# lukechencqu/quadrupedal_foothold_planner

Hardware: AMD Instinct MI355X
Metric: footholds/sec (4 legs x N cycles x B poses) on 1k^2 @2cm map; `value` = device-resident (poses and every product stay in HBM), `value_8d` / `ms_per_step_8d` = SURVEY 8(d)'s wall time of fpe_plan with host buffers, result D2H included (pinned destinations; pageable ones in value_survey_8d) (higher is better)
Workload: dtype f64; 1 GPU; headline: 1000x1000 @2cm rough terrain (seed 1), B=4096 poses/GPU (seed 6), trot, 8 cycles, searchRadius 0.1, all products written; `value` is device-resident (inputs and results stay in HBM; the PCIe-inclusive rate is value_incl_d2h); poses_per_gpu=4096, n_cycles=8, generator=synth-1, kernels=bit-window where supported, exchange=none

## Files before the change

### quadrupedal_foothold_planner_amd/csrc/fpe_bits_lane8.hpp

```cpp
#pragma once

namespace {


struct Unit {
    float eA[9];
    float eB[9];
    float eC;
    uint32_t pad0;
    uint32_t visA, visB;
    int nomRow, nomCol;
    uint32_t nomFlags;
    int cenRow, cenCol;
    uint32_t cenCode;
    double cx;
    double cenX;
    double defX;
    uint32_t pad[2];
};
static_assert(sizeof(Unit) == 144 && sizeof(Unit) % 16 == 0 && offsetof(Unit, visA) == 80 && offsetof(Unit, cx) == 112, "Unit layout");

template <bool kWant>
__device__ __forceinline__ void unit_put_disc(const DevMap& m, const PlanConsts& pc, double cx, double cy, const BBox& bb,
                                              const Grp<8>& g, const DiscLoads& d, float* e, uint32_t& vis, float* scratch) {
// ... 320 lines not shown
        c.xlo = nx2 - r;
        c.yhi = ny + 0.5 * r;
        c.ylo = ny - 0.5 * r;
    }
    c.vx = sh.polyX[leg];
    c.vy = sh.polyY[leg];
    c.footDa = sh.footDa;
    c.footDb = sh.footDb;
    c.footOff = sh.footOff;
    c.R2 = lk.R2;
    c.nRings = lk.nRings;
    c.nCand = lk.nCand;
    c.ti0 = c.tj0 = 0;
    c.ici = c.icj = 0;

    NominalOut no;
    CentroidOut co;
    float zDefault = static_cast<float>(static_cast<double>(0.0f) + pc.h);
    float* scratch = reinterpret_cast<float*>(lb.a);
    const bool wantDefault = out.default_next != nullptr;
    const bool usable = (ye.flags & 2) != 0 && fabs(c.cx) <= 1e6;
    if (!ls.radiusOk || !usable) {
        nominal_invalid(no, c.cx, c.cy, ls.radiusOk ? 2 : 3);
        co.x = co.y = 0.0; co.z = 0.0f; co.row = co.col = -1; co.code = 6;
        if (wantDefault && centre_usable(nx0, ny)) {
            const BBox dbox = circle_bbox_fast(m.g, nx0, ny, pc.rf);
            bool unused;
            zDefault = disc_pass_direct<G, false>(m, pc, nx0, ny, dbox, g, unused, scratch);
        }
        if constexpr (kMid) {
            if (g.sub == 0) {
                unit->visA = 0x80000000u;
                unit->eA[0] = 0.0f;
                unit->visB = 0x80000000u;
                unit->eB[0] = zDefault;
                unit->eC = 0.0f;
            }
        } else {
            ugFlags = kUgPreA | kUgPreB;
            ugVisA = __float_as_uint(0.0f);
            ugVisB = __float_as_uint(zDefault);
        }
    } else {
        const int q = g.sub;
        const double cq = (q == 5 || q == 6) ? nx0 : c.cx;
        const bool rawq = q == 4 || q == 7;
        const double hq = (q == 2 || q == 3) ? 0.5 * lk.lx : (rawq ? 0.0 : pc.rf);
        const bool minus = q == 1 || q == 3 || q == 6;
        const double xq = rawq ? cq : (minus ? cq - hq : cq + hq);
        int idxq;
        bool withinq = true;
        {
            const double n = (xq - m.g.orgX) - m.g.posX;
            const double qf = n * m.g.rinv;
            const double k = trunc(qf);
            const double fr = fabs(qf - k);
            bool safe = fr > pc.cornerEps && fr < 1.0 - pc.cornerEps;
            if (!rawq) safe = safe && qf < -pc.cornerEps && qf > pc.cornerEps - static_cast<double>(m.g.rows);
            idxq = -static_cast<int>(k);
            if (__ballot(!safe) != 0ull) {
                const Box bq{cq, 0.0, hq, 0.0};
                const CornerVal cv = corner_quantity(m.g, minus ? 2 : 0, bq, rawq);
                idxq = cv.idx;
                withinq = cv.within;
            }
        }
        constexpr int kKeep = (~(G - 1)) & 0x1F;
        BBox bb, rbox, dbox;
        bb.i0 = __builtin_amdgcn_ds_swizzle(idxq, kKeep | (0 << 5));
        bb.ni = __builtin_amdgcn_ds_swizzle(idxq, kKeep | (1 << 5)) - bb.i0 + 1;
        rbox.i0 = __builtin_amdgcn_ds_swizzle(idxq, kKeep | (2 << 5));
        rbox.ni = __builtin_amdgcn_ds_swizzle(idxq, kKeep | (3 << 5)) - rbox.i0 + 1;
        c.ici = __builtin_amdgcn_ds_swizzle(idxq, kKeep | (4 << 5));
        dbox.i0 = __builtin_amdgcn_ds_swizzle(idxq, kKeep | (5 << 5));
        dbox.ni = __builtin_amdgcn_ds_swizzle(idxq, kKeep | (6 << 5)) - dbox.i0 + 1;
        bb.j0 = dbox.j0 = ye.j0d;
        bb.nj = dbox.nj = ye.njd;
        rbox.j0 = ye.j0r;
        rbox.nj = ye.njr;
        c.icj = ye.jc;
        const unsigned wbits = static_cast<unsigned>(g.ballot(withinq));
        Submap sm;
        sm.i0 = rbox.i0;
        sm.j0 = rbox.j0;
        sm.ni = rbox.ni;
        sm.nj = rbox.nj;
        {
            const bool okX = (wbits & 0xCu) == 0xCu && sm.i0 >= 0 && sm.i0 < m.g.rows && sm.i0 + sm.ni <= m.g.rows;
            const double cornerX = cell_pos(m.g.baseX, m.g.res, sm.i0) - (-(0.5 * m.g.res));
            const double subLenX = static_cast<double>(sm.ni) * m.g.res;
            const double subOrgX = 0.5 * subLenX;
            const double subPosX = cornerX - subOrgX;
            sm.ok = okX && (ye.flags & 1) != 0 && within_axis(c.cx, subOrgX, subPosX, subLenX);
            sm.baseX = sm.ok ? subPosX + (subOrgX - 0.5 * m.g.res) : 0.0;
            sm.baseY = sm.ok ? ye.sbaseY : 0.0;
        }
        const int iw0 = c.ici - pc.winH, jw0 = c.icj - pc.winH;
        uint4 grp[NRL][KW + 1];
        win_issue<G, NRL, KW>(bm, m.g, g, iw0, jw0, grp);
        DiscLoads dc, dd;
        const bool dfltUsable = wantDefault && fabs(nx0) <= 1e6;
        uint32_t rowA = 0u, rowB = 0u;
        bool rowsA = false, rowsB = false;
        if constexpr (kMid) {
            disc_issue<G, false, kMid, kMid>(m, pc, c.cx, c.cy, bb, g, dc, ye.dy2);
            if (dfltUsable) disc_issue<G, false, kMid, kMid>(m, pc, nx0, ny, dbox, g, dd, ye.dy2);
        } else {
            dc.pipelined = dd.pipelined = false;
            dc.mid = dd.mid = false;
            const bool fitA = bb.ni <= 8 && bb.nj <= 8 && bb.ni * bb.nj <= 32;
            const bool fitB = !dfltUsable || (dbox.ni <= 8 && dbox.nj <= 8 && dbox.ni * dbox.nj <= 32);
            rowsA = __ballot(!fitA) == 0ull;
            rowsB = __ballot(!fitB) == 0ull;
            if (rowsA || rowsB) disc_rows8(m.g, pc.rf2, c.cx, nx0, c.cy, bb, dbox, g, rowA, rowB);
        }
        WinRows<NRL, KW> w;
        win_finish<NRL, KW>(jw0, grp, w);
#pragma unroll
        for (int k = 0; k < NRL; ++k) lb.a[g.sub + G * k] = w.Df[k][0];
        const CentroidScan sc = rows_from_bits<G, NRL, KW>(sm, w, g, iw0, jw0);
        bits_sync<G>();
        bool defaultOk;
        if constexpr (kMid) {
            defaultOk = default_ok_bits<G, KW, kMid>(m, pc, c.cx, c.cy, bb, dc, lb.a, lb.rows, iw0, jw0, g);
        } else {
            defaultOk = rowsA ? default_ok_rows8(rowA, bb, lb.a, lb.rows, iw0, jw0, g)
                              : default_ok_bits<G, KW, kMid>(m, pc, c.cx, c.cy, bb, dc, lb.a, lb.rows, iw0, jw0, g);
        }
        bits_sync<G>();
        float zCentre = 0.0f;
        if constexpr (kMid) {
            uint32_t visA = 0u, visB = 0u;
            unit_put_disc<true>(m, pc, c.cx, c.cy, bb, g, dc, unit->eA, visA, scratch);
            if (dfltUsable) unit_put_disc<true>(m, pc, nx0, ny, dbox, g, dd, unit->eB, visB, scratch);
            if (g.sub == 0) {
                unit->visA = visA;
                unit->visB = visB;
            }
        } else {
            bool pre;
            if (rowsA) {
                ugVisA = box_mask_from_rows8(rowA, bb.nj, g);
            } else {
                unitg_put_disc(m, pc, c.cx, c.cy, bb, g, dc, ugVisA, pre, scratch);
                if (pre) ugFlags |= kUgPreA;
            }
            ugAI0 = bb.i0; ugAJ0 = bb.j0; ugANj = max(bb.nj, 1);
            if (dfltUsable) {
                if (rowsB) {
                    ugVisB = box_mask_from_rows8(rowB, dbox.nj, g);
                } else {
                    unitg_put_disc(m, pc, nx0, ny, dbox, g, dd, ugVisB, pre, scratch);
                    if (pre) ugFlags |= kUgPreB;
                }
                ugBI0 = dbox.i0; ugBJ0 = dbox.j0; ugBNj = max(dbox.nj, 1);
            } else {
                ugFlags |= kUgPreB;
                ugVisB = __float_as_uint(zDefault);
            }
        }
        constexpr bool kOneCell = kMid;
        CentroidPendingBits cp;
        centroid_begin_bits<kOneCell>(m, c, sm, sc, zCentre, cp, ye.yA, ye.yB);
        if (defaultOk) {
            no.valid = 1;
            no.source = 0;
            no.row = c.ici;
            no.col = c.icj;
            no.x = c.cx;
            no.y = c.cy;
            no.z = zCentre;
        } else {
            nominal_invalid(no, c.cx, c.cy, 2);
            int wi = 0, wj = 0;
            bits_sync<G>();
            if (spiral_bits<G, NRL, KW, kMid>(m, pc, lut, head, c, w, lb, g, iw0, jw0, wi, wj, &ye)) {
                no.valid = 1;
                no.source = 1;
                no.row = wi;
                no.col = wj;
                no.x = cell_pos(m.g.baseX, m.g.res, wi);
                no.y = cell_pos(m.g.baseY, m.g.res, wj);
                no.z = zCentre;
            }
            bits_sync<G>();
        }
        if constexpr (kMid) {
            if (g.sub == 0) unit->eC = cp.e0;
            cp.o.z = 0.0f;
            if (g.sub == 0) unit->cenCode = static_cast<uint32_t>(cp.o.code) | (cp.needDisc != 0 ? 0x100u : 0u);
        } else {
            cp.o.z = 0.0f;
            if (cp.needDisc != 0) ugFlags |= kUgCTable;
            else if (cp.o.code == 0) ugFlags |= kUgCIsA;
        }
        co = cp.o;
    }
    lc->valid = no.valid;
    lc->v[0][0] = nx0;   lc->v[0][1] = ny;    lc->v[0][2] = static_cast<double>(zDefault);
    lc->v[1][0] = co.x;  lc->v[1][1] = co.y;  lc->v[1][2] = static_cast<double>(co.z);
    lc->v[2][0] = no.x;  lc->v[2][1] = no.y;  lc->v[2][2] = static_cast<double>(no.z);
    if constexpr (!kMid) {
        if (g.sub == 0) {
            UnitG u;
            u.cx = c.cx; u.cenX = co.x; u.defX = nx0;
            u.aI0 = ugAI0; u.aJ0 = ugAJ0; u.visA = ugVisA;
            u.bI0 = ugBI0; u.bJ0 = ugBJ0; u.visB = ugVisB;
            u.nomRow = no.row; u.nomCol = no.col; u.cenRow = co.row; u.cenCol = co.col;
            u.flags = static_cast<uint32_t>(co.code) | (no.valid ? kUgValid : 0u) | (static_cast<uint32_t>(no.source) << kUgSrcShift) | ugFlags |
                      (static_cast<uint32_t>(ugANj) << 16) | (static_cast<uint32_t>(ugBNj) << 24);
            u.pad[0] = u.pad[1] = u.pad[2] = 0u;
            *unit = u;
        }
    } else {
        if (g.sub == 0) {
            unit->nomRow = no.row;
            unit->nomCol = no.col;
            unit->nomFlags = static_cast<uint32_t>(no.valid) | (static_cast<uint32_t>(no.source) << 8);
            unit->cenRow = co.row;
            unit->cenCol = co.col;
            if (!(!ls.radiusOk || !usable)) {
            } else {
                unit->cenCode = static_cast<uint32_t>(co.code);
            }
            unit->cx = c.cx;
            unit->cenX = co.x;
            unit->defX = nx0;
        }
    }
}

struct HotConsts {
    double rf, rf2, cornerEps, oneMinusEps, drift;
};
struct LaneRole {
    double hqS;
    double qLo, qHi;
};
__device__ __forceinline__ int lane_track(int q) { return (q == 5 || q == 6) ? 0 : (q == 7 ? 2 : 1); }
__device__ __forceinline__ LaneRole make_lane_role(int q, double rf, double lx, double cornerEps, double rowsD) {
    LaneRole r;
    const double inf = __builtin_huge_val();
    const bool raw = q == 4 || q == 7;
    const double h = (q == 2 || q == 3) ? 0.5 * lx : (raw ? 0.0 : rf);
    const bool minus = q == 1 || q == 3 || q == 6;
    r.hqS = in_vgpr(minus ? -h : h);
    r.qLo = in_vgpr(raw ? -inf : cornerEps - rowsD);
    r.qHi = in_vgpr(raw ? inf : -cornerEps);
    return r;
}
struct FastRanks {
    uint32_t rowTab;
    int slot;
    unsigned long long di, dj;
};
template <int NRL>
__device__ __forceinline__ FastRanks load_fast_ranks(const SpiralLut& lut, const Grp<8>& g, int winH) {
    FastRanks fr;
    fr.slot = 0;
    int d = 99;
#pragma unroll
    for (int k = 0; k < NRL; ++k) {
        const int dk = g.sub + 8 * k - winH;
        const bool mine = dk >= -2 && dk <= 2;
        fr.slot = mine ? k : fr.slot;
        d = mine ? dk : d;
    }
    const uint32_t w = lut.fast16[min(max(d + 2, 0), 4)];
    fr.rowTab = d == 99 ? 0x1FFFFFFu : w;
    fr.di = *reinterpret_cast<const unsigned long long*>(lut.fast16 + 6);
    fr.dj = *reinterpret_cast<const unsigned long long*>(lut.fast16 + 8);
    asm volatile("" : "+v"(fr.di), "+v"(fr.dj));
    return fr;
}

struct MidKernArgs {
    const fpe_pose* poses;
    int B, nCycles;
    DevMap m;
    BitMap bm;
    PlanMidConsts pc;
    SpiralLut lut;
    fpe_plan_out out;
};
__device__ __forceinline__ const MidKernArgs* mid_cold_args() {
    typedef const MidKernArgs __attribute__((address_space(4))) * KernArgPtr;
    KernArgPtr ka4 = (KernArgPtr)__builtin_amdgcn_kernarg_segment_ptr();
    asm volatile("" : "+s"(ka4));
    return (const MidKernArgs*)ka4;
}
__device__ __forceinline__ PlanConsts plan_consts_of(const PlanMidConsts& k) {
    PlanConsts pc{};
    pc.rf = k.rf;
    pc.rf2 = k.rf2;
    pc.h = k.h;
    pc.winH = k.winH;
    pc.cornerEps = k.cornerEps;
    pc.nFoot = 1;
    pc.footReach = 0;
    pc.midCellInside = k.midCellInside;
    return pc;
}

template <int NRL, bool kNoDefault, int kProd, bool kPlain>
__device__ __forceinline__ void leg_fast8m(const DevMap& m, const BitMap& bm, int winH, bool wantDefaultArg, const HotConsts& hc, const LaneRole& role,
                                           const FastRanks& fk,
                                           const LutHead& head, PoseShared& sh, const LegBits& lb, const Grp<8>& g,
                                           int leg, const LegStatic& ls, const YEntry& yeIn, double myCtr, double advance, int cyc,
                                           LegCommit* lc, Unit* unit) {
    constexpr int G = 8, KW = 1;
    const LegConst& lk = ls.lk;
    const YEntry& yeLds = yeIn;
    YEntry ye;
    ye.jc = yeLds.jc; ye.j0d = yeLds.j0d; ye.njd = yeLds.njd; ye.j0r = yeLds.j0r;
    ye.njr = yeLds.njr; ye.jA = yeLds.jA; ye.jB = yeLds.jB; ye.flags = yeLds.flags;
    ye.ny = yeLds.ny; ye.sbaseY = yeLds.sbaseY; ye.yA = yeLds.yA; ye.yB = yeLds.yB;
    ye.rmask = yeLds.rmask; ye.pmask = yeLds.pmask;
    const double nxq = (myCtr + advance) + ls.biasX;
    const double ny = ye.ny;
    const bool wantDefault = kNoDefault ? false : wantDefaultArg;
    const double xq = nxq + role.hqS;
    const double qf = ((xq - m.g.orgX) - m.g.posX) * m.g.rinv;
    const double kq = trunc(qf);
    const double fr = fabs(qf - kq);
    const bool safe = (fr > hc.cornerEps && fr < hc.oneMinusEps && qf < role.qHi && qf > role.qLo) || g.sub == 7;
    const int idxq = -static_cast<int>(kq);
    constexpr int kKeep = (~(G - 1)) & 0x1F;
    const int i0d = bcast8_dpp<0>(idxq);
    const int i1d = bcast8_dpp<1>(idxq);
    const int i0r = bcast8_dpp<2>(idxq);
    const int i1r = bcast8_dpp<3>(idxq);
    const int ici = bcast8_dpp<4>(idxq);
    const int i0f = bcast8_dpp<5>(idxq);
    const int i1f = bcast8_dpp<6>(idxq);
    const double cx = bcast8_dpp_f64<0>(nxq);
    const double nx0 = bcast8_dpp_f64<5>(nxq);
    const double nx2 = bcast8_dpp_f64<7>(nxq);
    const int j0d = ye.j0d, icj = ye.jc;
    const int iw0 = ici - winH, jw0 = icj - winH;
    uint4 grp[NRL][KW + 1];
    win_issue<G, NRL, KW>(bm, m.g, g, iw0, jw0, grp);
    const int lowest = kNoDefault ? min(i0d, j0d) : min(min(i0d, i0f), j0d), lastRow = (kNoDefault ? i0d : max(i0d, i0f)) + 4;
    const bool boxF = kNoDefault ? true : ((i1f - i0f) == 2);
    const bool boxes = ((i1d - i0d) == 2) & boxF & (ye.njd == 3) & (lowest >= 1) & (lastRow <= m.g.rows) & (j0d + 4 <= m.g.cols);
    const bool dfltLane = (g.sub == 5) | (g.sub == 6);
    const bool laneOk = kNoDefault ? (dfltLane | (safe & (fabs(nxq) <= 1e6))) : (safe & (fabs(nxq) <= 1e6));
    const bool rare = (!kPlain & !ls.radiusOk) | ((ye.flags & (2 | kYCentreMid)) != (2 | kYCentreMid)) | !laneOk | (!kNoDefault & !wantDefault) | !boxes;
    if (__ballot(rare) != 0ull) {
        const double ctr0 = swizzle_f64<kKeep | (5 << 5)>(myCtr), ctr1 = swizzle_f64<kKeep | (0 << 5)>(myCtr),
                     ctr2 = swizzle_f64<kKeep | (7 << 5)>(myCtr);
        const MidKernArgs* ka = mid_cold_args();
        const PlanConsts pcR = plan_consts_of(ka->pc);
        const fpe_plan_out outR = specialise_products<kProd>(ka->out);
        leg_phase_bits8<NRL, true>(m, bm, pcR, ka->lut, head, sh, lb, g, leg, ls, yeIn, ctr0, ctr1, ctr2, advance, cyc, outR, lc, unit);
        return;
    }
    Submap sm;
    sm.i0 = i0r;
    sm.j0 = ye.j0r;
    sm.ni = i1r - i0r + 1;
    sm.nj = ye.njr;
    {
        const double cornerX = cell_pos(m.g.baseX, m.g.res, sm.i0) - (-(0.5 * m.g.res));
        const double subLenX = static_cast<double>(sm.ni) * m.g.res;
        const double subOrgX = 0.5 * subLenX;
        const double subPosX = cornerX - subOrgX;
        sm.ok = (ye.flags & 1) != 0 && within_axis(cx, subOrgX, subPosX, subLenX);
        sm.baseX = subPosX + (subOrgX - 0.5 * m.g.res);
        sm.baseY = ye.sbaseY;
    }
    const int t = g.sub + (g.sub >= 4 ? 1 : 0);
    const int a = t >= 6 ? 2 : (t >= 3 ? 1 : 0);
    const int bq = t - 3 * a;
    const double dy2 = yeLds.dy2[bq];
    const double dxA = cell_pos(m.g.baseX, m.g.res, i0d + a) - cx;
    const double dxB = cell_pos(m.g.baseX, m.g.res, i0f + a) - nx0;
    const bool visA = (dxA * dxA + dy2) <= hc.rf2;
    const bool visB = kNoDefault ? false : (dxB * dxB + dy2) <= hc.rf2;
    const unsigned colsU = static_cast<unsigned>(m.g.cols);
    const unsigned laneCell = __umul24(static_cast<unsigned>(a), colsU) + static_cast<unsigned>(bq);
    const unsigned boxA = __umul24(static_cast<unsigned>(i0d), colsU) + static_cast<unsigned>(j0d);
    const unsigned boxB = __umul24(static_cast<unsigned>(i0f), colsU) + static_cast<unsigned>(j0d);
    const float eA = load_cell(m.elev, boxA + laneCell);
    const float eMidA = load_cell(m.elev, boxA + colsU + 1u);
    float eB = 0.0f, eMidB = 0.0f;
    if constexpr (!kNoDefault) {
        eB = load_cell(m.elev, boxB + laneCell);
        eMidB = load_cell(m.elev, boxB + colsU + 1u);
    }
    bool fastSpiral;
    if constexpr (kPlain) fastSpiral = lk.nRings >= 4 && lk.nCand >= 16;
    else fastSpiral = __ballot(ls.polyKind != 0 || lk.nRings < 4 || lk.nCand < 16) == 0ull;
    const int iFast = iw0 + g.sub + G * fk.slot;
    const double rS = static_cast<double>(ls.Rf);
    const double xFast = cell_pos(m.g.baseX, m.g.res, iFast);
    const bool rowInside = (xFast < nx2 + rS) & (xFast >= nx2 - rS);
    WinRows<NRL, KW> w;
    win_finish<NRL, KW>(jw0, grp, w);
    const CentroidScan sc = rows_from_bits<G, NRL, KW>(sm, w, g, iw0, jw0, &ye.rmask);
    const unsigned mA = static_cast<unsigned>(g.ballot(visA)), mB = kNoDefault ? 0u : static_cast<unsigned>(g.ballot(visB));
    const unsigned visA9 = (mA & 0xFu) | 0x10u | ((mA & 0xF0u) << 1), visB9 = kNoDefault ? 0u : ((mB & 0xFu) | 0x10u | ((mB & 0xF0u) << 1));
    bool fail = false;
    {
        const unsigned sh3 = static_cast<unsigned>(j0d - jw0) & 31u;
#pragma unroll
        for (int k = 0; k < NRL; ++k) {
            const int ar = g.sub + G * k - (i0d - iw0);
            const unsigned bitsRow = (visA9 >> (3u * (static_cast<unsigned>(ar) & 3u))) & 7u;
            const unsigned sel = static_cast<unsigned>(ar) < 3u ? bitsRow : 0u;
            fail |= (((w.Df[k][0] >> sh3) & 7u) & sel) != 0u;
        }
    }
    const bool defaultOk = !g.any(fail);
    unit->eA[t] = eA;
    unit->eA[4] = eMidA;
    if constexpr (!kNoDefault) {
        unit->eB[t] = eB;
        unit->eB[4] = eMidB;
    }
    const int bottomRow = sm.ni - 1, rightCol = sm.nj - 1;
    const int minRow = sc.minRow, maxRow = sc.maxRow;
    const bool top = minRow == 0, bottom = maxRow == bottomRow;
    const bool case1 = top && !bottom;
    const bool case2 = !top && !bottom;
    const bool upper = minRow >= (bottomRow - maxRow);
    const int code23 = upper ? 2 : 3, code51 = bottom ? 5 : 1;
    int code = bottom ? 4 : code23;
    code = top ? code51 : code;
    code = sc.whole ? 0 : code;
    code = sm.ok ? code : 6;
    const bool useMaxRow = case1 || (case2 && !upper);
    const int rowA = (maxRow + bottomRow + (case1 ? 1 : 0)) >> 1, rowB = (minRow + 1) >> 1;
    const int newRow = useMaxRow ? rowA : rowB;
    const int newCol = (rightCol + (case1 ? 1 : 0)) >> 1;
    const bool whole = code == 0;
    const bool hasCell = static_cast<unsigned>(code - 1) < 4u;
    CentroidOut co;
    co.code = code;
    co.z = 0.0f;
    const double cellX = cell_pos(sm.baseX, m.g.res, newRow);
    const double yAB = code == 1 ? ye.yA : ye.yB;
    const double xCell = hasCell ? cellX : 0.0, yCell = hasCell ? yAB : 0.0;
    const int rowCell = hasCell ? sm.i0 + newRow : -1, colCell = hasCell ? sm.j0 + newCol : -1;
    co.x = whole ? cx : xCell;
    co.y = whole ? ny : yCell;
    co.row = whole ? ici : rowCell;
    co.col = whole ? icj : colCell;
    NominalOut no;
    no.valid = 1;
    no.source = 0;
    no.row = ici;
    no.col = icj;
    no.x = cx;
    no.y = ny;
    no.z = 0.0f;
    if (!defaultOk) {
        nominal_invalid(no, cx, ny, 2);
        const double r = static_cast<double>(ls.Rf);
        int wi = 0, wj = 0;
        bool found = false, searched = false;
        if (fastSpiral) {
            unsigned Fs = w.F[0][0], Cs = w.C[0][0];
#pragma unroll
            for (int k = 1; k < NRL; ++k) {
                Fs = fk.slot == k ? w.F[k][0] : Fs;
                Cs = fk.slot == k ? w.C[k][0] : Cs;
            }
            const unsigned inside = rowInside ? ye.pmask : 0u;
            const unsigned P = ~Fs | (~Cs & inside);
            const unsigned b5 = P >> static_cast<unsigned>(winH - 2);
            unsigned m16 = 0u;
#pragma unroll
            for (int c = 0; c < 5; ++c) m16 |= ((b5 >> c) & 1u) << ((fk.rowTab >> (5 * c)) & 31u);
            const unsigned all16 = or_reduce8(m16) & 0xFFFFu;
            found = all16 != 0u;
            const unsigned rank4 = static_cast<unsigned>(__builtin_ctz(all16 | 0x10000u) & 15) * 4u;
            wi = ici + static_cast<int>((fk.di >> rank4) & 7ull) - 2;
            wj = icj + static_cast<int>((fk.dj >> rank4) & 7ull) - 2;
            searched = lk.nCand <= 16;
        }
        if (!found && !searched) {
            LegCtx c;
            c.cyc = cyc;
            c.cx = cx;
            c.cy = ny;
            c.nv = (kPlain || ls.polyKind == 0) ? 4 : 6;
            c.rect = kPlain || ls.polyKind == 0;
            c.xhi = nx2 + r;
            c.xlo = nx2 - r;
            c.yhi = ny + 0.5 * r;
            c.ylo = ny - 0.5 * r;
            c.vx = sh.polyX[leg];
            c.vy = sh.polyY[leg];
            c.footDa = sh.footDa;
            c.footDb = sh.footDb;
            c.footOff = sh.footOff;
            c.R2 = lk.R2;
            c.nRings = lk.nRings;
            c.nCand = lk.nCand;
            c.ti0 = c.tj0 = 0;
            c.ici = ici;
            c.icj = icj;
            if (!kPlain && !c.rect) {
                if (g.sub == 0) {
                    double* vx = sh.polyX[leg];
                    double* vy = sh.polyY[leg];
                    const double hx = 0.5 * r, hy = (0.5 * r) * 0.8660254037844386;
                    vx[0] = nx2 + r;   vy[0] = ny;
                    vx[1] = nx2 + hx;  vy[1] = ny - hy;
                    vx[2] = nx2 - hx;  vy[2] = ny - hy;
                    vx[3] = nx2 - r;   vy[3] = ny;
                    vx[4] = nx2 - hx;  vy[4] = ny + hy;
                    vx[5] = nx2 + hx;  vy[5] = ny + hy;
                }
                bits_sync<G>();
            }
            const MidKernArgs* ka = mid_cold_args();
            const PlanConsts pcR = plan_consts_of(ka->pc);
            found = spiral_bits<G, NRL, KW, true>(m, pcR, ka->lut, head, c, w, lb, g, iw0, jw0, wi, wj, &yeIn);
            bits_sync<G>();
        }
        if (found) {
            no.valid = 1;
            no.source = 1;
            no.row = wi;
            no.col = wj;
            no.x = cell_pos(m.g.baseX, m.g.res, wi);
            no.y = cell_pos(m.g.baseY, m.g.res, wj);
        }
    }
    if (g.sub == 0) {
        unit->visA = visA9;
        unit->visB = visB9;
        unit->nomRow = no.row;
        unit->nomCol = no.col;
        unit->nomFlags = static_cast<uint32_t>(no.valid) | (static_cast<uint32_t>(no.source) << 8);
        unit->cenRow = co.row;
        unit->cenCol = co.col;
        unit->cenCode = static_cast<uint32_t>(code) | (hasCell ? 0x200u : 0u);
        unit->cx = cx;
        unit->cenX = co.x;
        unit->defX = nx0;
    }
    lc->valid = no.valid;
    lc->v[0][0] = nx0;   lc->v[0][1] = ny;    lc->v[0][2] = 0.0;
    lc->v[1][0] = co.x;  lc->v[1][1] = co.y;  lc->v[1][2] = 0.0;
    lc->v[2][0] = no.x;  lc->v[2][1] = no.y;  lc->v[2][2] = 0.0;
}

}

constexpr int kBitsGenericWaves = 3;
template <int NRL, bool kMid, int kProd, bool kPlain, bool kStride = false, class PC>
__device__ __forceinline__ void plan_bits_body(const fpe_pose* pp, int b, bool live, double x0, double y0, double z0, int gait, float rOverride,
                                               int polyKindIn, int nCycles, const DevMap& m, const DevMap& mArg, const BitMap& bm, const PC& pc,
                                               const SpiralLut& lut, const fpe_plan_out& out, const HotConsts& hc, int tid, int slot, int leg,
                                               const StrideVals& sv = StrideVals{}) {
    static_assert(kMid || !kPlain, "the generic kernels have no plain instance");
    static_assert(!kMid || !kStride, "the 3x3-only kernels have no stride instance");
    constexpr int G = 8;
    constexpr bool kNoDefault = kProd == 1;
    constexpr int kPoseThreads = 4 * G;
    constexpr int NR = G * NRL;
    extern __shared__ __attribute__((aligned(16))) unsigned char smem[];
    const Grp<G> g(tid);
    const size_t legBytes = 4 * static_cast<size_t>(legbits_words(NR, 1, pc.nHW));
    constexpr int kBatch = kMid ? 8 : 4;
    using UnitT = typename std::conditional<kMid, Unit, UnitG>::type;
    const size_t poseBytes = sizeof(PoseShared) + 4 * legBytes + (sizeof(YEntry) + sizeof(UnitT)) * 4 * kBatch;
    unsigned char* base = smem + static_cast<size_t>(slot) * poseBytes;
    PoseShared& sh = *reinterpret_cast<PoseShared*>(base);
    const LegBits lb = make_legbits(base + sizeof(PoseShared) + static_cast<size_t>(leg) * legBytes, NR, 1);
    YEntry* ytab = reinterpret_cast<YEntry*>(base + sizeof(PoseShared) + 4 * legBytes) + leg * kBatch;
    UnitT* units = reinterpret_cast<UnitT*>(base + sizeof(PoseShared) + 4 * legBytes + sizeof(YEntry) * 4 * kBatch) + leg * kBatch;

    const LutHead head = load_lut_head(lut, g);
    LegStatic ls;
    {
        if (!kPlain && __ballot(rOverride > 0.0f) != 0ull) {
            ls = make_leg_static(pc, pp, leg, m.g.res, lut);
        } else {
            ls.Rf = pc.searchRadius;
            ls.polyKind = kPlain ? 0 : polyKindIn;
            ls.radiusOk = true;
            const double R = static_cast<double>(pc.searchRadius);
            ls.lk.Rf = pc.searchRadius;
            ls.lk.R2 = R * R;
            ls.lk.nRings = pc.defNRings;
            ls.lk.nCand = pc.defNCand;
            ls.lk.lx = static_cast<double>(pc.searchRadius * 2);
            ls.lk.ly = static_cast<double>(pc.searchRadius);
            const bool odd = (leg & 1) != 0, high = (leg & 2) != 0;
            const double bxLo = odd ? pc.biasX[1] : pc.biasX[0], bxHi = odd ? pc.biasX[3] : pc.biasX[2];
            const double byLo = odd ? pc.biasY[1] : pc.biasY[0], byHi = odd ? pc.biasY[3] : pc.biasY[2];
            ls.biasX = high ? bxHi : bxLo;
            ls.biasY = high ? byHi : byLo;
        }
    }
    if constexpr (kMid) {
        ls.biasX = in_vgpr(ls.biasX);
        ls.biasY = in_vgpr(ls.biasY);
    }
    if constexpr (kMid) {
        if (tid % kPoseThreads == 0) {
            sh.footDa[0] = 0;
            sh.footDb[0] = 0;
            sh.footOff[0] = 0;
        }
    } else {
        for (int k = tid % kPoseThreads; k < pc.nFoot; k += kPoseThreads) {
            sh.footDa[k] = pc.footDa[k];
            sh.footDb[k] = pc.footDb[k];
            sh.footOff[k] = 0;
        }
    }
    if (g.sub == 0) {
        double sx = (leg == 0 || leg == 3) ? pc.LbHalf : -pc.LbHalf;
        double sy = (leg <= 1) ? pc.WbHalfNeg : pc.WbHalfPos;
        double sz = 0;
        sx += x0;
        sy += y0;
        sz += z0;
        if (out.stance && live) {
            double* st = out.stance + (static_cast<size_t>(b) * 4 + leg) * 3;
            st[0] = sx;
            st[1] = sy;
            st[2] = sz;
        }
        for (int t = 0; t < 3; ++t) {
            sh.cur[t][leg][0] = sx - (kStride ? sv.stepHalf : pc.stepHalf);
            sh.cur[t][leg][1] = sy;
            sh.cur[t][leg][2] = sz;
        }
    }
    bits_sync<G>();
    constexpr bool kStanceOnce = kMid && NRL < 4;
    double stanceCtr = 0.0;
    if constexpr (kStanceOnce) stanceCtr = polygon_center_x(sh.cur[0]);
    if (out.pose_status) {
        const double gx = (kStanceOnce ? stanceCtr : polygon_center_x(sh.cur[0])) + (kStride ? sv.step : pc.step), gy = y0 + 0.0;
        Submap gs;
        {
            const bool isY = (g.sub & 1) != 0, isBR = (g.sub & 2) != 0;
            const double ctr = isY ? gy : gx, halfExt = isY ? 0.5 * pc.isosWid : 0.5 * pc.isosLen;
            const double org = isY ? m.g.orgY : m.g.orgX, pos = isY ? m.g.posY : m.g.posX;
            const double cells = isY ? static_cast<double>(mArg.g.cols) : static_cast<double>(mArg.g.rows);
            const double vq = isBR ? ctr - halfExt : ctr + halfExt;
            const double qf = ((vq - org) - pos) * m.g.rinv;
            const double kq = trunc(qf);
            const double fr = fabs(qf - kq);
            const bool safe = (fr > pc.cornerEps) & (fr < 1.0 - pc.cornerEps) & (qf < -pc.cornerEps) & (qf > pc.cornerEps - cells);
            if (__ballot(!safe) == 0ull) {
                const int idxq = -static_cast<int>(kq);
                constexpr int kKeep = (~(G - 1)) & 0x1F;
                BBox gbb;
                gbb.i0 = __builtin_amdgcn_ds_swizzle(idxq, kKeep | (0 << 5));
                gbb.j0 = __builtin_amdgcn_ds_swizzle(idxq, kKeep | (1 << 5));
                gbb.ni = __builtin_amdgcn_ds_swizzle(idxq, kKeep | (2 << 5)) - gbb.i0 + 1;
                gbb.nj = __builtin_amdgcn_ds_swizzle(idxq, kKeep | (3 << 5)) - gbb.j0 + 1;
                gs = submap_from_corners(m.g, gbb, true, gx, gy);
            } else {
                const Box gb{gx, gy, 0.5 * pc.isosLen, 0.5 * pc.isosWid};
                Corners<G, 8> gc;
                gc.eval(m.g, g, gb, gb, gb, gb, 0x0u);
                gs = submap_from_corners(m.g, gc.template bbox<0>(g), gc.box_within(0), gx, gy);
            }
        }
        if (live && leg == 0 && g.sub == 0)
            out.pose_status[b] = (centre_usable(gx, gy) && gs.ok) ? 0 : static_cast<uint8_t>(FPE_POSE_OPT_SUBMAP_FAILED);
    }

    double adjY = 0.0;
    const int nPhases = (!kPlain && gait == 1) ? 4 : 1;
    const double advance = (!kPlain && gait == 1) ? (kStride ? sv.stepQuarter : pc.stepQuarter) : (kStride ? sv.step : pc.step);
    const int walkOrder = pc.RF_FIRST ? ((0) | (2 << 2) | (3 << 4) | (1 << 6)) : ((3) | (1 << 2) | (0 << 4) | (2 << 6));
    constexpr int kPoseLanes = 4 * G;
    const unsigned long long poseMask = ((1ull << kPoseLanes) - 1ull) << (slot * kPoseLanes);
    const int myTrack = kMid ? lane_track(g.sub) : (g.sub < 2 ? g.sub : 2);
    LaneRole role{};
    if constexpr (kMid) role = make_lane_role(g.sub, pc.rf, ls.lk.lx, pc.cornerEps, static_cast<double>(mArg.g.rows));
    FastRanks fr{};
    if constexpr (kMid) fr = load_fast_ranks<NRL>(lut, g, pc.winH);
    const bool wantDefault = out.default_next != nullptr;
    uint32_t okBits = 0u;

    unsigned hwSlot = 0u;
    if constexpr (kMid) {
        asm volatile("s_getreg_b32 %0, hwreg(HW_REG_HW_ID)" : "=s"(hwSlot));
        hwSlot &= 15u;
    }
    constexpr int kPrioSwapEighths = 3;
    for (int cyc = 0; cyc < nCycles; ++cyc) {
        if (kMid && cyc == (nCycles * kPrioSwapEighths) / 8 && (hwSlot & 1u)) __builtin_amdgcn_s_setprio(2);
        if ((cyc & (kBatch - 1)) == 0) {
            double a = adjY, mine = adjY;
#pragma unroll
            for (int k = 1; k < kBatch; ++k) {
                a += hc.drift;
                if (g.sub == k) mine = a;
            }
            if constexpr (kMid) {
                const YFillConsts yc{hc.rf, hc.cornerEps, pc.winH};
                fill_yentry(m.g, yc, ls, (y0 + mine) + ls.biasY, ytab[g.sub]);
            } else if (g.sub < kBatch) {
                fill_yentry(m.g, pc, ls, (y0 + mine) + ls.biasY, ytab[g.sub]);
            }
            bits_sync<G>();
        }
        const YEntry& ye = ytab[cyc & (kBatch - 1)];
        bool cycleOk = true;
        for (int ph = 0; ph < nPhases; ++ph) {
            const unsigned mask = (!kPlain && gait == 1) ? (1u << ((walkOrder >> (2 * ph)) & 3)) : 0xFu;
            const bool active = kPlain || ((mask >> leg) & 1u) != 0u;
            double myCtr = stanceCtr;
            if (!kStanceOnce || cyc != 0 || ph != 0) myCtr = polygon_center_x(sh.cur[myTrack]);
            LegCommit lc;
            lc.valid = 1;
            if (active) {
                if constexpr (kMid) {
                    leg_fast8m<NRL, kNoDefault, kProd, kPlain>(m, bm, pc.winH, wantDefault, hc, role, fr, head, sh, lb, g, leg, ls, ye, myCtr, advance, cyc, &lc,
                                                       units + (cyc & (kBatch - 1)));
                } else {
                    constexpr int kKeep = (~(G - 1)) & 0x1F;
                    const double ctr0 = swizzle_f64<kKeep | (0 << 5)>(myCtr), ctr1 = swizzle_f64<kKeep | (1 << 5)>(myCtr),
                                 ctr2 = swizzle_f64<kKeep | (2 << 5)>(myCtr);
                    leg_phase_bits8<NRL, false>(m, bm, pc, lut, head, sh, lb, g, leg, ls, ye, ctr0, ctr1, ctr2, advance, cyc, out, &lc,
                                                units + (cyc & (kBatch - 1)));
                }
            }
            const bool phaseOk = (__ballot(lc.valid == 0) & poseMask) == 0ull;
            if (phaseOk && active && g.sub == 0) {
#pragma unroll
                for (int t = 0; t < 3; ++t) {
                    sh.cur[t][leg][0] = lc.v[t][0];
                    sh.cur[t][leg][1] = lc.v[t][1];
                }
            }
            bits_sync<G>();
            cycleOk = cycleOk && phaseOk;
        }
        adjY += hc.drift;
        okBits |= (cycleOk ? 1u : 0u) << (cyc & 7);
        if ((cyc & (kBatch - 1)) == kBatch - 1 || cyc == nCycles - 1) {
            const int c0 = cyc & ~(kBatch - 1);
            if constexpr (kMid) {
                const MidKernArgs* ka = mid_cold_args();
                const double hF = ka->pc.h;
                const fpe_plan_out outF = specialise_products<kProd>(ka->out);
                if (live && c0 + g.sub <= cyc) flush_unit(m, hF, units[g.sub], ytab[g.sub], b, c0 + g.sub, leg, nCycles, okBits, outF);
            } else {
                const int us = g.sub >> 1;
                if (live && c0 + us <= cyc)
                    flush_unit_g(m, pc, sh.footDa, sh.footDb, units[us], ytab[us], b, c0 + us, leg, g.sub & 1, nCycles, okBits, out);
            }
            okBits = 0u;
            bits_sync<G>();
        }
    }
}

template <int NRL, bool kMid, int kProd>
__global__ __launch_bounds__(64, kMid ? 2 : kBitsGenericWaves) void plan_bits_kernel(const fpe_pose* __restrict__ poses, int B, int nCycles,
                                                          DevMap mArg, BitMap bm, typename std::conditional<kMid, PlanMidConsts, PlanConsts>::type pc,
                                                          SpiralLut lut, fpe_plan_out outArg) {
    constexpr int G = 8;
    const fpe_plan_out out = specialise_products<kProd>(outArg);
    constexpr int kPoseThreads = 4 * G;
    const int tid = static_cast<int>(threadIdx.x);
    const int slot = tid / kPoseThreads;
    const int leg = (tid / G) & 3;
    int b = blockIdx.x * 2 + slot;
    const bool live = b < B;
    if (!live) b = B - 1;
    const fpe_pose* pp = poses + b;
    const double x0 = pp->position[0], y0 = pp->position[1], z0 = pp->position[2];
    const int gait = pp->gait;
    const float rOverride = pp->leg_search_radius[leg];
    const int polyKindIn = pp->leg_polygon_kind[leg];
    __builtin_amdgcn_sched_barrier(0);
    DevMap m = mArg;
    if constexpr (kMid) {
        m.g.res = in_vgpr(m.g.res);
        m.g.rinv = in_vgpr(m.g.rinv);
        m.g.lenX = in_vgpr(m.g.lenX);
        m.g.lenY = in_vgpr(m.g.lenY);
        m.g.posX = in_vgpr(m.g.posX);
        m.g.posY = in_vgpr(m.g.posY);
        m.g.orgX = in_vgpr(m.g.orgX);
        m.g.orgY = in_vgpr(m.g.orgY);
        m.g.baseX = in_vgpr(m.g.baseX);
        m.g.baseY = in_vgpr(m.g.baseY);
    }
    HotConsts hc;
    hc.rf = in_vgpr(pc.rf);
    hc.rf2 = in_vgpr(pc.rf2);
    hc.cornerEps = in_vgpr(pc.cornerEps);
    hc.oneMinusEps = in_vgpr(1.0 - pc.cornerEps);
    hc.drift = kMid ? in_vgpr(pc.drift) : pc.drift;
    if constexpr (kMid) {
        if (__ballot(gait == 1 || rOverride > 0.0f || polyKindIn != 0) == 0ull) {
            plan_bits_body<NRL, kMid, kProd, true>(pp, b, live, x0, y0, z0, gait, rOverride, polyKindIn, nCycles, m, mArg, bm, pc, lut, out, hc, tid, slot,
                                                   leg);
            return;
        }
    }
    plan_bits_body<NRL, kMid, kProd, false>(pp, b, live, x0, y0, z0, gait, rOverride, polyKindIn, nCycles, m, mArg, bm, pc, lut, out, hc, tid, slot, leg);
}

static_assert(kernargs_mirror<decltype(plan_bits_kernel<2, true, 2>)>(
                  {offsetof(MidKernArgs, poses), offsetof(MidKernArgs, B), offsetof(MidKernArgs, nCycles), offsetof(MidKernArgs, m),
                   offsetof(MidKernArgs, bm), offsetof(MidKernArgs, pc), offsetof(MidKernArgs, lut), offsetof(MidKernArgs, out)},
                  offsetof(MidKernArgs, out) + sizeof(MidKernArgs::out)),
              "MidKernArgs must mirror the parameters of plan_bits_kernel<NRL, true, kProd>");

template <int NRL, int kProd>
__global__ __launch_bounds__(64, kBitsGenericWaves) void plan_bits_stride_kernel(const fpe_pose* __restrict__ poses, int B, int nCycles, DevMap mArg, BitMap bm,
                                                                                PlanConsts pc, SpiralLut lut, fpe_plan_out outArg,
                                                                                const fpe_stride* __restrict__ strides) {
    constexpr int G = 8;
    const fpe_plan_out out = specialise_products<kProd>(outArg);
    constexpr int kPoseThreads = 4 * G;
    const int tid = static_cast<int>(threadIdx.x);
    const int slot = tid / kPoseThreads;
    const int leg = (tid / G) & 3;
    int b = blockIdx.x * 2 + slot;
    const bool live = b < B;
    if (!live) b = B - 1;
    const fpe_pose* pp = poses + b;
    const double x0 = pp->position[0], y0 = pp->position[1], z0 = pp->position[2];
    const int gait = pp->gait;
    const float rOverride = pp->leg_search_radius[leg];
    const int polyKindIn = pp->leg_polygon_kind[leg];
    const StrideVals sv = load_stride(strides, b);
    __builtin_amdgcn_sched_barrier(0);
    HotConsts hc;
    hc.rf = in_vgpr(pc.rf);
    hc.rf2 = in_vgpr(pc.rf2);
    hc.cornerEps = in_vgpr(pc.cornerEps);
    hc.oneMinusEps = in_vgpr(1.0 - pc.cornerEps);
    hc.drift = sv.drift;
    plan_bits_body<NRL, false, kProd, false, true>(pp, b, live, x0, y0, z0, gait, rOverride, polyKindIn, nCycles, mArg, mArg, bm, pc, lut, out, hc, tid, slot, leg,
                                                   sv);
}
```

Baseline: 6.471 billion footholds/s.

## Split plain-path cycle loop into hot fast loop with cold fallback loop

For the plain kernel variant, the per-cycle loop becomes a hot loop that calls a specialised leg_fast8m, which bails out (returns true) on rare cases or when a full spiral search is needed. The rest of the batch then reruns in a cold loop that rebuilds leg bits and the LUT head from kernel arguments. This keeps the cold-path state (lb, head) out of the hot loop, cutting register pressure and code size there. The cost is a redo of the cycle that triggered the exit, plus extra code and recomputation on the fallback path. A profiling script counting hot-loop exits is added.

```diff
diff --git a/profiles/count_hot_loop_exits.py b/profiles/count_hot_loop_exits.py
--- /dev/null
+++ b/profiles/count_hot_loop_exits.py
@@ -0,0 +1,67 @@
+import os
+import sys
+
+import numpy as np
+
+sys.path.insert(0, os.path.join(os.path.dirname(os.path.abspath(__file__)), ".."))
+
+from oracle import fpo
+from quadrupedal_foothold_planner_amd import _capi, synth
+from tests import util
+from tests.test_gpu_hot_loop_exits import centres
+
+
+def count(name):
+    trav, elev, res, poses, n, extra = synth.make_config(name)
+    params = _capi.params_yaml()
+    if "search_radius" in extra:
+        params["searchRadius"] = np.float32(extra["search_radius"])
+    R = float(params["searchRadius"][0])
+    rows, cols = trav.shape
+    half_x = 0.5 * rows * res
+    omap = fpo.OracleMap(trav, elev, res)
+    ora = omap.plan(util.to_oracle_params(params), util.to_oracle_poses(poses), n, threads=os.cpu_count() or 1)
+    B = poses.shape[0]
+    ex = np.zeros((B, n), dtype=np.uint8)
+    legs = searching = 0
+    for b in range(B):
+        cx, ny, nx0 = centres(ora, b)
+        for c in range(n):
+            for leg in range(4):
+                rare = not (abs(cx[c, leg]) + R < half_x)
+                for x in (cx[c, leg], nx0[c, leg]):
+                    ok, i, j = omap.get_index(float(x), float(ny[c, leg])) if (abs(x) <= 1e6 and abs(ny[c, leg]) <= 1e6) else (False, 0, 0)
+                    rare |= (not ok) or i < 2 or i > rows - 3 or j < 2 or j > cols - 3
+                legs += 1
+                if rare:
+                    ex[b, c] |= 1
+                    continue
+                nom = ora["nominal"][b, c, leg]
+                if nom["valid"] == 0:
+                    searching += 1
+                    ex[b, c] |= 2
+                elif nom["source"] == 1:
+                    searching += 1
+                    first16 = {tuple(int(v) for v in q) for q in omap.spiral_cells(float(cx[c, leg]), float(ny[c, leg]), R, max_cells=16)}
+                    if (int(nom["row"]), int(nom["col"])) not in first16:
+                        ex[b, c] |= 2
+    if B % 2:
+        ex = np.concatenate([ex, ex[-1:]])
+    wave = ex[0::2] | ex[1::2]
+    pairs = wave.size
+    leave = wave != 0
+    in_full = np.zeros_like(leave)
+    for c in range(n):
+        in_full[:, c] = leave[:, c] | (in_full[:, c - 1] if c % 8 else False)
+    print(f"{name}: {B} poses, {n} cycles, {legs} legs of which {searching} search ({100.0 * searching / legs:.1f} %)")
+    print(f"  (wavefront, cycle) pairs: {pairs}; exit A in {int((wave & 1).astype(bool).sum())} ({100.0 * (wave & 1).astype(bool).mean():.3f} %), "
+          f"exit B in {int((wave & 2).astype(bool).sum())} ({100.0 * (wave & 2).astype(bool).mean():.3f} %), either in {int(leave.sum())} "
+          f"({100.0 * leave.mean():.3f} %)")
+    print(f"  wavefronts that leave the hot loop at least once: {int(leave.any(axis=1).sum())} of {wave.shape[0]} "
+          f"({100.0 * leave.any(axis=1).mean():.2f} %); pairs run in the full loop: {int(in_full.sum())} ({100.0 * in_full.mean():.3f} %), "
+          f"cycles redone (one per wavefront and batch that leaves): {sum(int(leave[:, c0:c0 + 8].any(axis=1).sum()) for c0 in range(0, n, 8))}")
+
+
+if __name__ == "__main__":
+    for name in sys.argv[1:] or ["headline", "cfg2"]:
+        count(name)
diff --git a/quadrupedal_foothold_planner_amd/csrc/fpe_bits_lane8.hpp b/quadrupedal_foothold_planner_amd/csrc/fpe_bits_lane8.hpp
--- a/quadrupedal_foothold_planner_amd/csrc/fpe_bits_lane8.hpp
+++ b/quadrupedal_foothold_planner_amd/csrc/fpe_bits_lane8.hpp
@@ -646,8 +646,8 @@
     return pc;
 }
 
-template <int NRL, bool kNoDefault, int kProd, bool kPlain>
-__device__ __forceinline__ void leg_fast8m(const DevMap& m, const BitMap& bm, int winH, bool wantDefaultArg, const HotConsts& hc, const LaneRole& role,
+template <int NRL, bool kNoDefault, int kProd, bool kPlain, bool kHot = false>
+__device__ __forceinline__ bool leg_fast8m(const DevMap& m, const BitMap& bm, int winH, bool wantDefaultArg, const HotConsts& hc, const LaneRole& role,
                                            const FastRanks& fk,
                                            const LutHead& head, PoseShared& sh, const LegBits& lb, const Grp<8>& g,
                                            int leg, const LegStatic& ls, const YEntry& yeIn, double myCtr, double advance, int cyc,
@@ -691,13 +691,14 @@
     const bool laneOk = kNoDefault ? (dfltLane | (safe & (fabs(nxq) <= 1e6))) : (safe & (fabs(nxq) <= 1e6));
     const bool rare = (!kPlain & !ls.radiusOk) | ((ye.flags & (2 | kYCentreMid)) != (2 | kYCentreMid)) | !laneOk | (!kNoDefault & !wantDefault) | !boxes;
     if (__ballot(rare) != 0ull) {
+        if constexpr (kHot) return true;
         const double ctr0 = swizzle_f64<kKeep | (5 << 5)>(myCtr), ctr1 = swizzle_f64<kKeep | (0 << 5)>(myCtr),
                      ctr2 = swizzle_f64<kKeep | (7 << 5)>(myCtr);
         const MidKernArgs* ka = mid_cold_args();
         const PlanConsts pcR = plan_consts_of(ka->pc);
         const fpe_plan_out outR = specialise_products<kProd>(ka->out);
         leg_phase_bits8<NRL, true>(m, bm, pcR, ka->lut, head, sh, lb, g, leg, ls, yeIn, ctr0, ctr1, ctr2, advance, cyc, outR, lc, unit);
-        return;
+        return false;
     }
     Submap sm;
     sm.i0 = i0r;
@@ -733,7 +734,8 @@
         eMidB = load_cell(m.elev, boxB + colsU + 1u);
     }
     bool fastSpiral;
-    if constexpr (kPlain) fastSpiral = lk.nRings >= 4 && lk.nCand >= 16;
+    if constexpr (kHot) fastSpiral = true;
+    else if constexpr (kPlain) fastSpiral = lk.nRings >= 4 && lk.nCand >= 16;
     else fastSpiral = __ballot(ls.polyKind != 0 || lk.nRings < 4 || lk.nCand < 16) == 0ull;
     const int iFast = iw0 + g.sub + G * fk.slot;
     const double rS = static_cast<double>(ls.Rf);
@@ -798,6 +800,7 @@
     no.x = cx;
     no.y = ny;
     no.z = 0.0f;
+    bool needFull = false;
     if (!defaultOk) {
         nominal_invalid(no, cx, ny, 2);
         const double r = static_cast<double>(ls.Rf);
@@ -823,7 +826,9 @@
             wj = icj + static_cast<int>((fk.dj >> rank4) & 7ull) - 2;
             searched = lk.nCand <= 16;
         }
-        if (!found && !searched) {
+        if constexpr (kHot) {
+            needFull = !found && !searched;
+        } else if (!found && !searched) {
             LegCtx c;
             c.cyc = cyc;
             c.cx = cx;
@@ -873,6 +878,9 @@
             no.y = cell_pos(m.g.baseY, m.g.res, wj);
         }
     }
+    if constexpr (kHot) {
+        if (__ballot(needFull) != 0ull) return true;
+    }
     if (g.sub == 0) {
         unit->visA = visA9;
         unit->visB = visB9;
@@ -890,6 +898,7 @@
     lc->v[0][0] = nx0;   lc->v[0][1] = ny;    lc->v[0][2] = 0.0;
     lc->v[1][0] = co.x;  lc->v[1][1] = co.y;  lc->v[1][2] = 0.0;
     lc->v[2][0] = no.x;  lc->v[2][1] = no.y;  lc->v[2][2] = 0.0;
+    return false;
 }
 
 }
@@ -914,11 +923,13 @@
     const size_t poseBytes = sizeof(PoseShared) + 4 * legBytes + (sizeof(YEntry) + sizeof(UnitT)) * 4 * kBatch;
     unsigned char* base = smem + static_cast<size_t>(slot) * poseBytes;
     PoseShared& sh = *reinterpret_cast<PoseShared*>(base);
-    const LegBits lb = make_legbits(base + sizeof(PoseShared) + static_cast<size_t>(leg) * legBytes, NR, 1);
+    LegBits lb{};
+    if constexpr (!kPlain) lb = make_legbits(base + sizeof(PoseShared) + static_cast<size_t>(leg) * legBytes, NR, 1);
     YEntry* ytab = reinterpret_cast<YEntry*>(base + sizeof(PoseShared) + 4 * legBytes) + leg * kBatch;
     UnitT* units = reinterpret_cast<UnitT*>(base + sizeof(PoseShared) + 4 * legBytes + sizeof(YEntry) * 4 * kBatch) + leg * kBatch;
 
-    const LutHead head = load_lut_head(lut, g);
+    LutHead head{};
+    if constexpr (!kPlain) head = load_lut_head(lut, g);
     LegStatic ls;
     {
         if (!kPlain && __ballot(rOverride > 0.0f) != 0ull) {
@@ -1034,6 +1045,87 @@
         hwSlot &= 15u;
     }
     constexpr int kPrioSwapEighths = 3;
+    if constexpr (kPlain) {
+        int cyc = 0;
+        while (cyc < nCycles) {
+            {
+                double a = adjY, mine = adjY;
+#pragma unroll
+                for (int k = 1; k < kBatch; ++k) {
+                    a += hc.drift;
+                    if (g.sub == k) mine = a;
+                }
+                const YFillConsts yc{hc.rf, hc.cornerEps, pc.winH};
+                fill_yentry(m.g, yc, ls, (y0 + mine) + ls.biasY, ytab[g.sub]);
+                bits_sync<G>();
+            }
+            const int c0 = cyc;
+            const int cEnd = min(cyc + kBatch, nCycles);
+            const bool hotOk = (kNoDefault || wantDefault) && ls.lk.nRings >= 4 && ls.lk.nCand >= 16;
+            for (; hotOk && cyc < cEnd; ++cyc) {
+                if (cyc == (nCycles * kPrioSwapEighths) / 8 && (hwSlot & 1u)) __builtin_amdgcn_s_setprio(2);
+                double myCtr = stanceCtr;
+                if (!kStanceOnce || cyc != 0) myCtr = polygon_center_x(sh.cur[myTrack]);
+                LegCommit lc;
+                if (leg_fast8m<NRL, kNoDefault, kProd, true, true>(m, bm, pc.winH, wantDefault, hc, role, fr, head, sh, lb, g, leg, ls,
+                                                                   ytab[cyc & (kBatch - 1)], myCtr, advance, cyc, &lc, units + (cyc & (kBatch - 1))))
+                    break;
+                const bool cycleOk = (__ballot(lc.valid == 0) & poseMask) == 0ull;
+                if (cycleOk && g.sub == 0) {
+#pragma unroll
+                    for (int t = 0; t < 3; ++t) {
+                        sh.cur[t][leg][0] = lc.v[t][0];
+                        sh.cur[t][leg][1] = lc.v[t][1];
+                    }
+                }
+                bits_sync<G>();
+                adjY += hc.drift;
+                okBits |= (cycleOk ? 1u : 0u) << (cyc & 7);
+            }
+            if (cyc < cEnd) {
+                const MidKernArgs* ka = mid_cold_args();
+                int tidF = tid;
+                asm volatile("" : "+v"(tidF));
+                const int slotF = tidF / kPoseThreads, legF = (tidF / G) & 3;
+                const size_t legBytesF = 4 * static_cast<size_t>(legbits_words(NR, 1, ka->pc.nHW));
+                const size_t poseBytesF = sizeof(PoseShared) + 4 * legBytesF + (sizeof(YEntry) + sizeof(UnitT)) * 4 * kBatch;
+                const LegBits lbF = make_legbits(smem + static_cast<size_t>(slotF) * poseBytesF + sizeof(PoseShared) + static_cast<size_t>(legF) * legBytesF, NR, 1);
+                const LutHead headF = load_lut_head(ka->lut, g);
+                LegStatic lsF = ls;
+                {
+                    const double R = static_cast<double>(ka->pc.searchRadius);
+                    lsF.lk.R2 = R * R;
+                }
+                for (; cyc < cEnd; ++cyc) {
+                    if (cyc == (nCycles * kPrioSwapEighths) / 8 && (hwSlot & 1u)) __builtin_amdgcn_s_setprio(2);
+                    const double myCtr = polygon_center_x(sh.cur[myTrack]);
+                    LegCommit lc;
+                    leg_fast8m<NRL, kNoDefault, kProd, true, false>(m, bm, pc.winH, wantDefault, hc, role, fr, headF, sh, lbF, g, legF, lsF,
+                                                                    ytab[cyc & (kBatch - 1)], myCtr, advance, cyc, &lc, units + (cyc & (kBatch - 1)));
+                    const bool cycleOk = (__ballot(lc.valid == 0) & poseMask) == 0ull;
+                    if (cycleOk && g.sub == 0) {
+#pragma unroll
+                        for (int t = 0; t < 3; ++t) {
+                            sh.cur[t][leg][0] = lc.v[t][0];
+                            sh.cur[t][leg][1] = lc.v[t][1];
+                        }
+                    }
+                    bits_sync<G>();
+                    adjY += hc.drift;
+                    okBits |= (cycleOk ? 1u : 0u) << (cyc & 7);
+                }
+            }
+            {
+                const MidKernArgs* ka = mid_cold_args();
+                const double hF = ka->pc.h;
+                const fpe_plan_out outF = specialise_products<kProd>(ka->out);
+                if (live && c0 + g.sub < cEnd) flush_unit(m, hF, units[g.sub], ytab[g.sub], b, c0 + g.sub, leg, nCycles, okBits, outF);
+                okBits = 0u;
+                bits_sync<G>();
+            }
+        }
+        return;
+    }
     for (int cyc = 0; cyc < nCycles; ++cyc) {
         if (kMid && cyc == (nCycles * kPrioSwapEighths) / 8 && (hwSlot & 1u)) __builtin_amdgcn_s_setprio(2);
         if ((cyc & (kBatch - 1)) == 0) {
```

Result: no change. 6.535 billion footholds/s, median of 6 (+1.0%).
